# mom-ocean/MOM6

Measured on AMD Instinct MI355X. Metric: simulated-days/wall-sec, higher is better.
Workload: dtype f64

## Files before the change

mom6_amd/csrc/barotropic.hip:

```cpp
#include <algorithm>
#include <type_traits>
#include <vector>
#include <cmath>
#include "mom6x_dev.h"

void halo_wrap(mom6x_ctx *c, double *const *fields, const int *staggers, const int *nks, int n);

enum BTW {
  W_q = 0, W_DCor_u, W_DCor_v, W_gtot_E, W_gtot_W, W_gtot_N, W_gtot_S, W_eta, W_eta_PF,
  W_Cor_ref_u, W_Cor_ref_v, W_BT_force_u, W_BT_force_v, W_ubt, W_vbt, W_bt_rem_u, W_bt_rem_v,
  W_uhbt0, W_vhbt0, W_ubt_Cor, W_vbt_Cor, W_uhbt, W_vhbt, W_u_accel_bt, W_v_accel_bt,
  W_eta_src, W_e_anom, W_eta_sum, W_eta_wtd, W_ubt_wtd, W_vbt_wtd, W_eta_pred,
  W_uh0sum, W_vh0sum, W_ubt0, W_vbt0,
  W_f4u, W_f4u_2, W_f4u_3, W_f4u_4, W_f4v, W_f4v_2, W_f4v_3, W_f4v_4,
  W_BTCu,
  W_BTCv = W_BTCu + 10,
  W_BTtmp = W_BTCv + 10,
  W_uhn = W_BTtmp + 12,
  W_vhn,
  W_ubt2, W_vbt2, W_eta_pred2,
  W_COUNT
};

enum BTC { B_FA_EE = 0, B_FA_E0, B_FA_W0, B_FA_WW, B_uBT_WW, B_uBT_EE, B_crvW, B_crvE, B_uh_WW, B_uh_EE };
// ... 119 lines not shown
        if (e_k <= D_shallow) hat = h_harm;
        else {
          const double wt_arith = (e_k - D_shallow) / (h_arith + h_neglect);
          hat = wt_arith * h_arith + (1.0 - wt_arith) * h_harm;
        }
      }
      fr[c + k * slab] = hat;
      hattot = hattot + hat;
      e_below = e_k;
    }
    const double Ihattot = mC / (hattot + h_neglect);
    for (int k = 0; k < nz; k++) fr[c + k * slab] = fr[c + k * slab] * Ihattot;
  }
}

__global__ void k_bt_mass_source(Dm d, const double *__restrict__ G, const double *__restrict__ h,
                                 const double *__restrict__ eta, double *eta_cor, int set_cor, double Z_to_H) {
  const int i = blockIdx.x * blockDim.x + threadIdx.x, j = blockIdx.y * blockDim.y + threadIdx.y;
  if (i > d.ni - 1 || j > d.nj - 1) return;
  const size_t c = ix2(d, i, j);
  double eta_h = h[c] - gm(G, d, MOM6X_G_bathyT)[c] * Z_to_H;
  for (int k = 1; k < d.nk; k++) eta_h = eta_h + h[c + (size_t)k * d.slab];
  const double d_eta = eta_h - eta[c];
  eta_cor[c] = set_cor ? d_eta : (eta_cor[c] + d_eta);
}

__global__ void k_bt_mass_source_from(Dm d, const double *__restrict__ eta_h, const double *__restrict__ eta, double *eta_cor, int set_cor) {
  const int i = blockIdx.x * blockDim.x + threadIdx.x, j = blockIdx.y * blockDim.y + threadIdx.y;
  if (i > d.ni - 1 || j > d.nj - 1) return;
  const size_t c = ix2(d, i, j);
  const double d_eta = eta_h[c] - eta[c];
  eta_cor[c] = set_cor ? d_eta : (eta_cor[c] + d_eta);
}

__global__ void k_set_dtbt(Dm d, const double *__restrict__ G, const double *__restrict__ pbce,
                           const double *__restrict__ frhatu, const double *__restrict__ frhatv,
                           double gtot_est, double Z_to_H, double zadd, int add_max, double bebt, double cor_scale2,
                           double *Idt_max2_out, const double *__restrict__ eta) {
  const int i = blockIdx.x * blockDim.x + threadIdx.x, j = blockIdx.y * blockDim.y + threadIdx.y;
  if (i > d.ni - 1 || j > d.nj - 1) return;
  const int st = d.pitch;
  const size_t c = ix2(d, i, j), slab = (size_t)d.slab;
  const double *bathyT = gm(G, d, MOM6X_G_bathyT), *dy_Cu = gm(G, d, MOM6X_G_dy_Cu), *dx_Cv = gm(G, d, MOM6X_G_dx_Cv);
  const double *IdxCu = gm(G, d, MOM6X_G_IdxCu), *IdyCv = gm(G, d, MOM6X_G_IdyCv), *f2 = gm(G, d, MOM6X_G_Coriolis2Bu);
  double DatuE, DatuW, DatvN, DatvS;
  if (add_max) {
    DatuE = dy_Cu[c] * Z_to_H * dmax(dmax(bathyT[c + 1], bathyT[c]) + zadd, 0.0);
    DatuW = dy_Cu[c - 1] * Z_to_H * dmax(dmax(bathyT[c], bathyT[c - 1]) + zadd, 0.0);
    DatvN = dx_Cv[c] * Z_to_H * dmax(dmax(bathyT[c + st], bathyT[c]) + zadd, 0.0);
    DatvS = dx_Cv[c - st] * Z_to_H * dmax(dmax(bathyT[c], bathyT[c - st]) + zadd, 0.0);
  } else {
    auto Hc = [&](size_t x) { return eta ? (bathyT[x] * Z_to_H + eta[x]) : ((bathyT[x] + zadd) * Z_to_H); };
    const double H0 = Hc(c), HE = Hc(c + 1), HW = Hc(c - 1);
    const double HN = Hc(c + st), HS = Hc(c - st);
    DatuE = 0.0; if ((H0 > 0.0) && (HE > 0.0)) DatuE = dy_Cu[c] * (2.0 * H0 * HE) / (H0 + HE);
    DatuW = 0.0; if ((HW > 0.0) && (H0 > 0.0)) DatuW = dy_Cu[c - 1] * (2.0 * HW * H0) / (HW + H0);
    DatvN = 0.0; if ((H0 > 0.0) && (HN > 0.0)) DatvN = dx_Cv[c] * (2.0 * H0 * HN) / (H0 + HN);
    DatvS = 0.0; if ((HS > 0.0) && (H0 > 0.0)) DatvS = dx_Cv[c - st] * (2.0 * HS * H0) / (HS + H0);
  }
  double gE = gtot_est, gW = gtot_est, gN = gtot_est, gS = gtot_est;
  if (pbce) {
    gE = gW = gN = gS = 0.0;
    for (int k = 0; k < d.nk; k++) {
      const double pb = pbce[c + k * slab];
      gE = gE + pb * frhatu[c + k * slab];
      gW = gW + pb * frhatu[c - 1 + k * slab];
      gN = gN + pb * frhatv[c + k * slab];
      gS = gS + pb * frhatv[c - st + k * slab];
    }
  }
  Idt_max2_out[c] = 0.5 * (1.0 + 2.0 * bebt) * (gm(G, d, MOM6X_G_IareaT)[c] *
      (((gE * DatuE * IdxCu[c]) + (gW * DatuW * IdxCu[c - 1])) + ((gN * DatvN * IdyCv[c]) + (gS * DatvS * IdyCv[c - st]))) +
      ((f2[c] + f2[c - 1 - st]) + (f2[c - 1] + f2[c - st])) * cor_scale2);
}

struct ColArgs {
  const double *visc_rem, *frhat, *U_Cor, *pbce, *uh0, *u_uh0, *U_in, *bc_accel, *tau, *tau_bot, *IDat;
  const double *hf; double h_neglect;
  double *ubt_Cor, *gtot_m , *gtot_p , *uh0sum, *ubt0, *ubt, *BT_force, *bt_rem;
  double Instep, RZ_to_H, vel_underflow;
  int nstep, wt_uv_bug, visc_rem_u_uh0, strong_drag;
};

template <int DIR, bool HF>
__global__ void __launch_bounds__(256)
k_bt_col(Dm d, const double *__restrict__ G, ColArgs A) {
  const int i = I_BASE((DIR ? 0 : -1)) + blockIdx.x * blockDim.x + threadIdx.x;
  const int j = (DIR ? -1 : 0) + blockIdx.y * blockDim.y + threadIdx.y;
  if (i > d.ni - 1 || j > d.nj - 1) return;
  if (i < ((DIR ? 0 : -1))) return;
  const int st = DIR ? d.pitch : 1, nz = d.nk;
  const size_t c = ix2(d, i, j), slab = (size_t)d.slab;
  const double subroundoff = 1e-30;
  const double mC = gm(G, d, DIR ? MOM6X_G_mask2dCv : MOM6X_G_mask2dCu)[c];
  double Ihattot = 0.0;
  if (HF) {
    double hattot = 0.0;
    for (int k = 0; k < nz; k++) hattot = hattot + A.hf[c + (size_t)k * slab];
    Ihattot = mC / (hattot + A.h_neglect);
  }
#define FRH(k) (HF ? A.hf[c + (size_t)(k) * slab] * Ihattot : A.frhat[c + (size_t)(k) * slab])
  double Iwt_tot = 1.0;
  if (!A.wt_uv_bug) {
    double tot = 0.0;
    for (int k = 0; k < nz; k++) {
      double vr = dmin(A.visc_rem[c + k * slab], 1.);
      vr = dmax(vr, 1. - 0.5 * A.Instep / (vr + subroundoff));
      vr = dmax(vr, 0.);
      const double w = FRH(k) * vr;
      tot = (k == 0) ? w : (tot + w);
    }
    Iwt_tot = tot;
    if (fabs(tot) > 0.0) Iwt_tot = mC / tot;
  }
  double ubt_Cor = 0.0, gm_ = 0.0, gp_ = 0.0, uh0sum = 0.0, ubt0 = 0.0, ubt = 0.0, av_rem = 0.0;
  double BT_force = 0.0;
  if (mC > 0.0) {
    BT_force = A.tau[c] * A.RZ_to_H * A.IDat[c] * A.visc_rem[c];
    if (A.tau_bot) BT_force = BT_force - A.tau_bot[c] * A.RZ_to_H * A.IDat[c];
  }
  for (int k = 0; k < nz; k++) {
    const size_t f = c + k * slab;
    const double vrem = A.visc_rem[f], frh = FRH(k);
    double vr = dmin(vrem, 1.);
    vr = dmax(vr, 1. - 0.5 * A.Instep / (vr + subroundoff));
    vr = dmax(vr, 0.);
    double wt = frh * vr;
    if (!A.wt_uv_bug) wt = wt * Iwt_tot;
    ubt_Cor = ubt_Cor + wt * A.U_Cor[f];
    gm_ = gm_ + A.pbce[f] * wt;
    gp_ = gp_ + A.pbce[f + st] * wt;
    if (A.uh0) {
      uh0sum = uh0sum + A.uh0[f];
      ubt0 = ubt0 + (A.visc_rem_u_uh0 ? wt : frh) * A.u_uh0[f];
    }
    ubt = ubt + wt * A.U_in[f];
    BT_force = BT_force + wt * A.bc_accel[f];
    av_rem = av_rem + frh * vrem;
  }
#undef FRH
  A.ubt_Cor[c] = ubt_Cor;
  A.gtot_m[c] = gm_;
  A.gtot_p[c + st] = gp_;
  if (A.uh0) { A.uh0sum[c] = uh0sum; A.ubt0[c] = ubt0; }
  if (fabs(ubt) < A.vel_underflow) ubt = 0.0;
  A.ubt[c] = ubt;
  A.BT_force[c] = BT_force;
  double bt_rem;
  if (A.strong_drag) {
    bt_rem = mC * ((A.nstep * av_rem) / (1.0 + (A.nstep - 1) * av_rem));
  } else {
    bt_rem = 0.0;
    if (mC * av_rem > 0.0) bt_rem = mC * pow(av_rem, A.Instep);
  }
  A.bt_rem[c] = bt_rem;
}

__global__ void k_btcont_copy(Dm d, mom6x_BT_cont BT, double *tmp) {
  const int i = -1 + blockIdx.x * blockDim.x + threadIdx.x;
  const int j = -1 + blockIdx.y * blockDim.y + threadIdx.y;
  if (i > d.ni - 1 || j > d.nj - 1) return;
  const size_t c = ix2(d, i, j), slab = (size_t)d.slab;
  if (j >= 0) {
    tmp[0 * slab + c] = BT.uBT_EE[c]; tmp[1 * slab + c] = BT.uBT_WW[c]; tmp[2 * slab + c] = BT.FA_u_EE[c];
    tmp[3 * slab + c] = BT.FA_u_E0[c]; tmp[4 * slab + c] = BT.FA_u_W0[c]; tmp[5 * slab + c] = BT.FA_u_WW[c];
  }
  if (i >= 0) {
    tmp[6 * slab + c] = BT.vBT_NN[c]; tmp[7 * slab + c] = BT.vBT_SS[c]; tmp[8 * slab + c] = BT.FA_v_NN[c];
    tmp[9 * slab + c] = BT.FA_v_N0[c]; tmp[10 * slab + c] = BT.FA_v_S0[c]; tmp[11 * slab + c] = BT.FA_v_SS[c];
  }
}
__global__ void k_face_areas_as_fits(Dm d, const double *__restrict__ G, double Z_ref, double Z_to_H, double *tmp, const double *__restrict__ eta) {
  const int i = -2 + blockIdx.x * blockDim.x + threadIdx.x;
  const int j = -2 + blockIdx.y * blockDim.y + threadIdx.y;
  if (i > d.ni || j > d.nj) return;
  const int st = d.pitch;
  const size_t c = ix2(d, i, j), slab = (size_t)d.slab;
  const double *bathyT = gm(G, d, MOM6X_G_bathyT);
  const double H1 = eta ? (bathyT[c] * Z_to_H + eta[c]) : ((bathyT[c] + Z_ref) * Z_to_H);
  if (j >= -1) {
    const double H2 = eta ? (bathyT[c + 1] * Z_to_H + eta[c + 1]) : ((bathyT[c + 1] + Z_ref) * Z_to_H);
    double Dat = 0.0;
    if ((H1 > 0.0) && (H2 > 0.0)) Dat = gm(G, d, MOM6X_G_dy_Cu)[c] * (2.0 * H1 * H2) / (H1 + H2);
    tmp[0 * slab + c] = -1.0e100; tmp[1 * slab + c] = 1.0e100;
    tmp[2 * slab + c] = Dat; tmp[3 * slab + c] = Dat; tmp[4 * slab + c] = Dat; tmp[5 * slab + c] = Dat;
  }
  if (i >= -1) {
    const double H2 = eta ? (bathyT[c + st] * Z_to_H + eta[c + st]) : ((bathyT[c + st] + Z_ref) * Z_to_H);
    double Dat = 0.0;
    if ((H1 > 0.0) && (H2 > 0.0)) Dat = gm(G, d, MOM6X_G_dx_Cv)[c] * (2.0 * H1 * H2) / (H1 + H2);
    tmp[6 * slab + c] = -1.0e100; tmp[7 * slab + c] = 1.0e100;
    tmp[8 * slab + c] = Dat; tmp[9 * slab + c] = Dat; tmp[10 * slab + c] = Dat; tmp[11 * slab + c] = Dat;
  }
}
__global__ void k_face_areas_eta(Dm d, const double *__restrict__ G, double Z_to_H, const double *__restrict__ eta, double *Bu, double *Bv,
                                 int isv, int iev, int jsv, int jev) {
  const int i = isv - 2 + blockIdx.x * blockDim.x + threadIdx.x;
  const int j = jsv - 2 + blockIdx.y * blockDim.y + threadIdx.y;
  if (i > iev + 1 || j > jev + 1) return;
  const int st = d.pitch;
  const size_t c = ix2(d, i, j), slab = (size_t)d.slab;
  const double *bathyT = gm(G, d, MOM6X_G_bathyT);
  const double H1 = bathyT[c] * Z_to_H + eta[c];
  if (j >= jsv - 1) {
    const double H2 = bathyT[c + 1] * Z_to_H + eta[c + 1];
    double Dat = 0.0;
    if ((H1 > 0.0) && (H2 > 0.0)) Dat = gm(G, d, MOM6X_G_dy_Cu)[c] * (2.0 * H1 * H2) / (H1 + H2);
    Bu[B_FA_EE * slab + c] = Dat; Bu[B_FA_E0 * slab + c] = Dat; Bu[B_FA_W0 * slab + c] = Dat; Bu[B_FA_WW * slab + c] = Dat;
  }
  if (i >= isv - 1) {
    const double H2 = bathyT[c + st] * Z_to_H + eta[c + st];
    double Dat = 0.0;
    if ((H1 > 0.0) && (H2 > 0.0)) Dat = gm(G, d, MOM6X_G_dx_Cv)[c] * (2.0 * H1 * H2) / (H1 + H2);
    Bv[B_FA_EE * slab + c] = Dat; Bv[B_FA_E0 * slab + c] = Dat; Bv[B_FA_W0 * slab + c] = Dat; Bv[B_FA_WW * slab + c] = Dat;
  }
}
__global__ void k_btcl(Dm d, const double *__restrict__ tmp, double *Bu, double *Bv, int hs) {
  const int i = -hs - 1 + blockIdx.x * blockDim.x + threadIdx.x;
  const int j = -hs - 1 + blockIdx.y * blockDim.y + threadIdx.y;
  if (i > d.ni - 1 + hs || j > d.nj - 1 + hs) return;
  const size_t c = ix2(d, i, j), slab = (size_t)d.slab;
  const double C1_3 = 1.0 / 3.0;
  for (int dir = 0; dir < 2; dir++) {
    if (dir == 0 && j < -hs) continue;
    if (dir == 1 && i < -hs) continue;
    const double *t = tmp + (size_t)(dir * 6) * slab;
    double *B = dir ? Bv : Bu;
    const double FA_EE = t[2 * slab + c], FA_E0 = t[3 * slab + c], FA_W0 = t[4 * slab + c], FA_WW = t[5 * slab + c];
    const double uBT_EE = 1.0 * t[0 * slab + c], uBT_WW = 1.0 * t[1 * slab + c];
    B[B_FA_EE * slab + c] = FA_EE; B[B_FA_E0 * slab + c] = FA_E0; B[B_FA_W0 * slab + c] = FA_W0; B[B_FA_WW * slab + c] = FA_WW;
    B[B_uBT_EE * slab + c] = uBT_EE; B[B_uBT_WW * slab + c] = uBT_WW;
    B[B_uh_EE * slab + c] = uBT_EE * (C1_3 * (2.0 * FA_E0 + FA_EE));
    B[B_uh_WW * slab + c] = uBT_WW * (C1_3 * (2.0 * FA_W0 + FA_WW));
    double crvW = 0.0, crvE = 0.0;
    if (fabs(uBT_WW) > 0.0) crvW = (C1_3 * (FA_WW - FA_W0)) / (uBT_WW * uBT_WW);
    if (fabs(uBT_EE) > 0.0) crvE = (C1_3 * (FA_EE - FA_E0)) / (uBT_EE * uBT_EE);
    B[B_crvW * slab + c] = crvW; B[B_crvE * slab + c] = crvE;
  }
// ... 371 lines not shown
                               dtA * ((s_un[ty][tx - 1] - s_un[ty][tx]) + (s_vn[ty - 1][tx] - s_vn[ty][tx]));
      work[(size_t)P.e_out * slab + c] = eta_PF_BT;
      if (A.find_etaav && (fabs(A.wt_accel2_next) > 0.0) && i >= 0 && i <= d.ni - 1 && j >= 0 && j <= d.nj - 1)
        work[W_eta_sum * slab + c] = work[W_eta_sum * slab + c] + A.wt_accel2_next * eta_PF_BT;
    }
    if (i >= 0 && i < d.ni && j >= 0 && j < d.nj) {
      const double bT = gm(G, d, MOM6X_G_bathyT)[c];
      if ((e < -Z_to_H * bT) && (gm(G, d, MOM6X_G_mask2dT)[c] > 0.0)) {
        atomicAdd(&warn[0], 1ULL);
        if (atomicCAS(&warn[1], 0ULL, 1ULL) == 0ULL) { warn_info[0] = e; warn_info[1] = -bT; warn_info[2] = (double)i; warn_info[3] = (double)j; }
      }
    }
  }
}

__global__ void k_bt_clip(Dm d, const double *__restrict__ G, double *work, double dt, double CFL_trunc,
                          int isv, int iev, int jsv, int jev) {
  const int i = isv - 1 + blockIdx.x * blockDim.x + threadIdx.x;
  const int j = jsv - 1 + blockIdx.y * blockDim.y + threadIdx.y;
  if (i > iev || j > jev) return;
  const int st = d.pitch;
  const size_t c = ix2(d, i, j), slab = (size_t)d.slab;
  const double *IareaT = gm(G, d, MOM6X_G_IareaT), *areaT = gm(G, d, MOM6X_G_areaT);
  if (j >= jsv) {
    const double dy = gm(G, d, MOM6X_G_dy_Cu)[c];
    double u = work[W_ubt * slab + c];
    if ((u * (dt * dy)) * IareaT[c + 1] < -CFL_trunc) u = (-0.95 * CFL_trunc) * (areaT[c + 1] / (dt * dy));
    else if ((u * (dt * dy)) * IareaT[c] > CFL_trunc) u = (0.95 * CFL_trunc) * (areaT[c] / (dt * dy));
    work[W_ubt * slab + c] = u;
  }
  if (i >= isv) {
    const double dx = gm(G, d, MOM6X_G_dx_Cv)[c];
    double v = work[W_vbt * slab + c];
    if ((v * (dt * dx)) * IareaT[c + st] < -CFL_trunc) v = (-0.9 * CFL_trunc) * (areaT[c + st] / (dt * dx));
    else if ((v * (dt * dx)) * IareaT[c] > CFL_trunc) v = (0.9 * CFL_trunc) * (areaT[c] / (dt * dx));
    work[W_vbt * slab + c] = v;
  }
}

__global__ void k_bt_post(Dm d, double *work, const double *__restrict__ eta_in, double *eta_out, double *etaav,
                          double dgeo_de, double I_sum_wt_accel, double I_sum_wt_eta) {
  const int i = blockIdx.x * blockDim.x + threadIdx.x, j = blockIdx.y * blockDim.y + threadIdx.y;
  if (i > d.ni - 1 || j > d.nj - 1) return;
  const size_t c = ix2(d, i, j), slab = (size_t)d.slab;
  if (etaav) etaav[c] = work[W_eta_sum * slab + c] * I_sum_wt_accel;
  work[W_e_anom * slab + c] = dgeo_de * (0.5 * (work[W_eta * slab + c] + eta_in[c]) - work[W_eta_PF * slab + c]);
  eta_out[c] = work[W_eta_wtd * slab + c] * I_sum_wt_eta;
}

__global__ void __launch_bounds__(256)
k_layer_accel(Dm d, const double *__restrict__ G, const double *__restrict__ work, const double *__restrict__ pbce,
              double *__restrict__ accel_layer_u, double *__restrict__ accel_layer_v, double accel_underflow) {
  const int i = I_BASE(-1) + blockIdx.x * blockDim.x + threadIdx.x;
  const int j = -1 + blockIdx.y * blockDim.y + threadIdx.y;
  if (i > d.ni - 1 || j > d.nj - 1) return;
  if (i < (-1)) return;
  const int st = d.pitch;
  const size_t c = ix2(d, i, j), slab = (size_t)d.slab;
  const int k0 = blockIdx.z * KCHUNK, k1 = min(k0 + KCHUNK, d.nk);
  const double *e_anom = work + W_e_anom * slab;
  const double ea = e_anom[c], ea_E = e_anom[c + 1], ea_N = e_anom[c + st];
  const double g_E = work[W_gtot_E * slab + c], g_W = work[W_gtot_W * slab + c + 1];
  const double g_N = work[W_gtot_N * slab + c], g_S = work[W_gtot_S * slab + c + st];
  const double ua = work[W_u_accel_bt * slab + c], va = work[W_v_accel_bt * slab + c];
  const double IdxCu = gm(G, d, MOM6X_G_IdxCu)[c], IdyCv = gm(G, d, MOM6X_G_IdyCv)[c];
  for (int k = k0; k < k1; k++) {
    const size_t c3 = c + (size_t)k * slab;
    const double pb = pbce[c3];
    if (j >= 0) {
      double a = (ua - (((pbce[c3 + 1] - g_W) * ea_E) - ((pb - g_E) * ea)) * IdxCu);
      if (fabs(a) < accel_underflow) a = 0.0;
      accel_layer_u[c3] = a;
    }
    if (i >= 0) {
      double a = (va - (((pbce[c3 + st] - g_S) * ea_N) - ((pb - g_N) * ea)) * IdyCv);
      if (fabs(a) < accel_underflow) a = 0.0;
      accel_layer_v[c3] = a;
    }
  }
}

}

void bt_defer_layer_accel(mom6x_ctx *c, bool on) { if (c->bts) c->bts->la_defer = on; }

void bt_defer_btcalc(mom6x_ctx *c, bool on) {
  static const bool eager = [] { const char *e = getenv("MOM6X_BTCALC"); return e && !strcmp(e, "eager"); }();
  if (c->bts) c->bts->fr_defer = on && !eager;
}
static void btcalc_from_faces(mom6x_ctx *c, const double *h_u, const double *h_v) {
  const Dm d = c->d;
  const dim3 b = blk2();
  if (d.nk <= COLS_NK_BOUND) {
#define BTC(NKT) do {                                                                                                                   \
    KLAUNCH(c, "k_btcalc<0>", (k_btcalc_cols<0, NKT>), grid3(nxa(d.ni + 1, -1), d.nj, 1, b), b, d, c->G, h_u, c->bts->frhatu, c->GV.H_subroundoff); \
    KLAUNCH(c, "k_btcalc<1>", (k_btcalc_cols<1, NKT>), grid3(d.ni, d.nj + 1, 1, b), b, d, c->G, h_v, c->bts->frhatv, c->GV.H_subroundoff); } while (0)
    COLS_NK_DISPATCH(d.nk, BTC);
#undef BTC
    return;
  }
  KLAUNCH(c, "k_btcalc<0>", k_btcalc<0>, grid3(nxa(d.ni + 1, -1), d.nj, 1, b), b, d, c->G, (const double *)nullptr, h_u, c->bts->frhatu,
          c->GV.H_subroundoff, c->GV.Z_to_H, 0);
  KLAUNCH(c, "k_btcalc<1>", k_btcalc<1>, grid3(d.ni, d.nj + 1, 1, b), b, d, c->G, (const double *)nullptr, h_v, c->bts->frhatv,
          c->GV.H_subroundoff, c->GV.Z_to_H, 0);
}
int bt_frhat_materialize(mom6x_ctx *c) {
  BTState *s = c->bts;
  if (!s || !s->fr_pending) return MOM6X_OK;
  HIPCHK(hipSetDevice(c->device));
  btcalc_from_faces(c, s->fr_hu, s->fr_hv);
  s->fr_pending = false;
  HIPCHK(hipGetLastError());
  return MOM6X_OK;
}

bool bt_layer_accel_src(mom6x_ctx *c, LayerAccelSrc *u, LayerAccelSrc *v) {
  BTState *s = c->bts;
  if (!s || !s->la_pending) return false;
  const size_t slab = (size_t)c->d.slab;
  const double *w = s->work;
  u->pbce = v->pbce = s->la_pbce; u->e_anom = v->e_anom = w + W_e_anom * slab;
  u->g_own = w + W_gtot_E * slab; u->g_nbr = w + W_gtot_W * slab; u->a2d = w + W_u_accel_bt * slab;
  v->g_own = w + W_gtot_N * slab; v->g_nbr = w + W_gtot_S * slab; v->a2d = w + W_v_accel_bt * slab;
  u->underflow = v->underflow = s->la_underflow;
  return true;
}

int bt_layer_accel_materialize(mom6x_ctx *c, double *accel_layer_u, double *accel_layer_v) {
  BTState *s = c->bts;
  REQUIRE(s && s->la_pending, MOM6X_EINVAL, "btstep_layer_accel: the deferred layer accelerations of the step's last btstep are gone "
          "(another btstep has run since)");
  HIPCHK(hipSetDevice(c->device));
  const Dm d = c->d;
  const dim3 b = blk2();
  KLAUNCH(c, "k_layer_accel", k_layer_accel, grid3(nxa(d.ni + 1, -1), d.nj + 1, nchunks(d.nk), b), b, d, c->G, (const double *)s->work,
          s->la_pbce, accel_layer_u, accel_layer_v, s->la_underflow);
  s->la_pending = false;
  HIPCHK(hipGetLastError());
  return MOM6X_OK;
}

void bt_state_free(mom6x_ctx *c) {
  if (!c->bts) return;
  BTState *s = c->bts;
  double *ptrs[] = { s->frhatu, s->frhatv, s->IDatu, s->IDatv, s->ubtav, s->vbtav, s->eta_cor, s->q_D, s->D_u_Cor,
                     s->D_v_Cor, s->work, s->warn_info };
  for (double *p : ptrs) (void)hipFree(p);
  (void)hipFree(s->warn);
  delete s;
  c->bts = nullptr;
}

extern "C" int mom6x_btstep_warnings(mom6x_ctx *c, int reset, long long *count, double *info) {
  REQUIRE(c && c->bts && count, MOM6X_EINVAL, "mom6x_btstep_warnings: barotropic_init has not been called");
  HIPCHK(hipSetDevice(c->device));
  HIPCHK(hipStreamSynchronize(c->stream));
  unsigned long long w[2];
  HIPCHK(hipMemcpy(w, c->bts->warn, sizeof(w), hipMemcpyDeviceToHost));
  *count = (long long)w[0];
  if (info) HIPCHK(hipMemcpy(info, c->bts->warn_info, 4 * sizeof(double), hipMemcpyDeviceToHost));
  if (reset) HIPCHK(hipMemset(c->bts->warn, 0, sizeof(w)));
  return MOM6X_OK;
}

extern "C" int mom6x_barotropic_init(mom6x_ctx *c, const mom6x_barotropic_params *p) {
  REQUIRE(c && p, MOM6X_EINVAL, "mom6x_barotropic_init: null argument");
// ... 119 lines not shown
  const Dm d = c->d;
  const dim3 b = blk2();
  BTState *s = c->bts;
  { const int rcm = bt_frhat_materialize(c); if (rcm) return rcm; }
  double *tmp = s->work + (size_t)W_eta_pred * d.slab;
  HIPCHK(hipMemsetAsync(tmp, 0, sizeof(double) * d.slab, c->stream));
  KLAUNCH(c, "k_set_dtbt", k_set_dtbt, grid3(d.ni, d.nj, 1, b), b, d, c->G, pbce, s->frhatu, s->frhatv, gtot_est,
                     c->GV.Z_to_H, c->bt.Z_ref + SSH_add, add_max, c->bt.bebt, c->bt.BT_Coriolis_scale * c->bt.BT_Coriolis_scale, tmp, eta);
  HIPCHK(hipGetLastError());
  std::vector<double> host((size_t)d.slab);
  HIPCHK(hipMemcpyAsync(host.data(), tmp, sizeof(double) * d.slab, hipMemcpyDeviceToHost, c->stream));
  HIPCHK(hipStreamSynchronize(c->stream));
  double min_max_dt2 = 1.0e38;
  for (int j = 0; j < d.nj; j++) for (int i = 0; i < d.ni; i++) {
    const double I2 = host[(size_t)(i + d.ioff) + (size_t)(j + d.joff) * d.pitch];
    if (I2 * min_max_dt2 > 1.0) min_max_dt2 = 1.0 / I2;
  }
  const double dgeo_de = 1.0 + fmax(0.0, c->bt.G_extra);
  double dtbt_max = sqrt(min_max_dt2 / dgeo_de);
  { int rc_ = comm_allreduce_scalar(c, &dtbt_max, 0); if (rc_) return rc_; }
  c->bt.dtbt = c->bt.dtbt_fraction * dtbt_max;
  if (dtbt_out) *dtbt_out = c->bt.dtbt;
  return MOM6X_OK;
}

extern "C" int mom6x_btstep(mom6x_ctx *c, const double *U_in, const double *V_in, const double *eta_in, double dt,
                            const double *bc_accel_u, const double *bc_accel_v, const double *taux, const double *tauy,
                            const double *pbce, const double *eta_PF_in, const double *U_Cor, const double *V_Cor,
                            double *accel_layer_u, double *accel_layer_v, double *eta_out, double *uhbtav,
                            double *vhbtav, const double *visc_rem_u, const double *visc_rem_v,
                            const mom6x_BT_cont *BT_cont, const double *taux_bot, const double *tauy_bot,
                            const double *uh0, const double *vh0, const double *u_uh0, const double *v_vh0,
                            double *etaav) {
  REQUIRE(c && c->bt_init, MOM6X_EINVAL, "btstep: Module MOM_barotropic must be initialized before it is used.");
  REQUIRE(U_in && V_in && eta_in && bc_accel_u && bc_accel_v && taux && tauy && pbce && eta_PF_in && U_Cor && V_Cor &&
          accel_layer_u && accel_layer_v && eta_out && uhbtav && vhbtav && visc_rem_u && visc_rem_v,
          MOM6X_EINVAL, "btstep: null mandatory array");
  const bool add_uh0 = (uh0 != nullptr);
  REQUIRE(!add_uh0 || (vh0 && u_uh0 && v_vh0), MOM6X_EINVAL,
          "btstep: vh0, u_uh0, and v_vh0 must be associated if uh0 is used.");
  REQUIRE((taux_bot != nullptr) == (tauy_bot != nullptr), MOM6X_EINVAL, "btstep: taux_bot and tauy_bot come together");
  HIPCHK(hipSetDevice(c->device));
  const Dm d = c->d;
  const mom6x_barotropic_params &P = c->bt;
  BTState *s = c->bts;
  double *work = s->work;
  const size_t slab = (size_t)d.slab;
  const dim3 b = blk2();
  hipStream_t st = c->stream;
  const int is = 0, ie = d.ni - 1, js = 0, je = d.nj - 1;

  const double Idt = 1.0 / dt;
  const bool evolving_face_areas = !BT_cont && P.nonlinear_continuity && P.nonlin_cont_update_period > 0;
  const int stencil = evolving_face_areas ? std::max(2, P.min_stencil) : ((P.min_stencil > 1) ? P.min_stencil : 1);
  const int num_cycles = (P.use_wide_halos && d.halo / stencil >= 1) ? d.halo / stencil : 1;
  const int isvf = is - (num_cycles - 1) * stencil, ievf = ie + (num_cycles - 1) * stencil;
  const int jsvf = js - (num_cycles - 1) * stencil, jevf = je + (num_cycles - 1) * stencil;
  REQUIRE(P.dtbt > 0.0, MOM6X_EINVAL, "btstep: dtbt must be positive (call set_dtbt or set params.dtbt)");
  const int nstep = (int)ceil(dt / P.dtbt - 0.0001);
  s->nstep_last = nstep;
  const double Instep = 1.0 / (double)nstep;
  const double dtbt = dt * Instep;
  const double dgeo_de = 1.0 + P.G_extra;

  HIPCHK(hipMemsetAsync(work, 0, (size_t)W_COUNT * slab * sizeof(double), st));
  KLAUNCH(c, "k_bt_copy_in", k_bt_copy_in, grid3(d.ni + 2 * d.halo + 1, d.nj + 2 * d.halo + 1, 1, b), b, d, work, eta_in,
                     eta_PF_in, s->q_D, s->D_u_Cor, s->D_v_Cor);

  ColArgs Au;
  memset(&Au, 0, sizeof(Au));
  Au.visc_rem = visc_rem_u; Au.frhat = s->frhatu; Au.U_Cor = U_Cor; Au.pbce = pbce; Au.uh0 = uh0; Au.u_uh0 = u_uh0;
  Au.U_in = U_in; Au.bc_accel = bc_accel_u; Au.tau = taux; Au.tau_bot = taux_bot; Au.IDat = s->IDatu;
  Au.ubt_Cor = work + W_ubt_Cor * slab; Au.gtot_m = work + W_gtot_E * slab; Au.gtot_p = work + W_gtot_W * slab;
  Au.uh0sum = work + W_uh0sum * slab; Au.ubt0 = work + W_ubt0 * slab; Au.ubt = work + W_ubt * slab;
  Au.BT_force = work + W_BT_force_u * slab; Au.bt_rem = work + W_bt_rem_u * slab;
  Au.Instep = Instep; Au.RZ_to_H = c->GV.RZ_to_H; Au.vel_underflow = P.vel_underflow; Au.nstep = nstep;
  Au.wt_uv_bug = P.wt_uv_bug; Au.visc_rem_u_uh0 = P.visc_rem_u_uh0; Au.strong_drag = P.strong_drag;
  ColArgs Av = Au;
  Av.visc_rem = visc_rem_v; Av.frhat = s->frhatv; Av.U_Cor = V_Cor; Av.uh0 = vh0; Av.u_uh0 = v_vh0; Av.U_in = V_in;
  Av.bc_accel = bc_accel_v; Av.tau = tauy; Av.tau_bot = tauy_bot; Av.IDat = s->IDatv;
  Av.ubt_Cor = work + W_vbt_Cor * slab; Av.gtot_m = work + W_gtot_N * slab; Av.gtot_p = work + W_gtot_S * slab;
  Av.uh0sum = work + W_vh0sum * slab; Av.ubt0 = work + W_vbt0 * slab; Av.ubt = work + W_vbt * slab;
  Av.BT_force = work + W_BT_force_v * slab; Av.bt_rem = work + W_bt_rem_v * slab;
  if (s->fr_pending) {
    Au.hf = s->fr_hu; Av.hf = s->fr_hv; Au.h_neglect = Av.h_neglect = c->GV.H_subroundoff;
    KLAUNCH(c, "k_bt_col<0>", (k_bt_col<0, true>), grid3(nxa(d.ni + 1, -1), d.nj, 1, b), b, d, c->G, Au);
    KLAUNCH(c, "k_bt_col<1>", (k_bt_col<1, true>), grid3(d.ni, d.nj + 1, 1, b), b, d, c->G, Av);
  } else {
    { const int rcm = bt_frhat_materialize(c); if (rcm) return rcm; }
    KLAUNCH(c, "k_bt_col<0>", (k_bt_col<0, false>), grid3(nxa(d.ni + 1, -1), d.nj, 1, b), b, d, c->G, Au);
    KLAUNCH(c, "k_bt_col<1>", (k_bt_col<1, false>), grid3(d.ni, d.nj + 1, 1, b), b, d, c->G, Av);
  }

  double *tmp = work + W_BTtmp * slab;
  if (BT_cont) KLAUNCH(c, "k_btcont_copy", k_btcont_copy, grid3(d.ni + 1, d.nj + 1, 1, b), b, d, *BT_cont, tmp);
  else KLAUNCH(c, "k_face_areas_as_fits", k_face_areas_as_fits, grid3(d.ni + 3, d.nj + 3, 1, b), b, d, c->G, P.Z_ref, c->GV.Z_to_H, tmp,
               P.nonlinear_continuity ? (const double *)(work + W_eta * slab) : (const double *)nullptr);
  {
    double *f[18]; int stg[18], nks[18];
    for (int m = 0; m < 12; m++) { f[m] = tmp + (size_t)m * slab; stg[m] = (m < 6) ? 1 : 2; nks[m] = 1; }
    double *g[] = { work + W_gtot_E * slab, work + W_gtot_N * slab, work + W_gtot_W * slab, work + W_gtot_S * slab,
                    work + W_ubt_Cor * slab, work + W_vbt_Cor * slab };
    const int gs[] = { 0, 0, 0, 0, 1, 2 };
    for (int m = 0; m < 6; m++) { f[12 + m] = g[m]; stg[12 + m] = gs[m]; nks[12 + m] = 1; }
    halo_wrap(c, f, stg, nks, 18);
  }
  const int hs = 1 + ievf - ie;
  KLAUNCH(c, "k_btcl", k_btcl, grid3(d.ni + 2 * hs + 1, d.nj + 2 * hs + 1, 1, b), b, d, tmp, work + W_BTCu * slab,
                     work + W_BTCv * slab, hs);
  if (add_uh0) KLAUNCH(c, "k_uhbt0", k_uhbt0, grid3(d.ni + 1, d.nj + 1, 1, b), b, d, work, work);

  KLAUNCH(c, "k_find_Cor", k_find_Cor, grid3(ievf - isvf + 3, jevf - jsvf + 3, 1, b), b, d, work, P.Sadourny, isvf, ievf, jsvf, jevf);
  KLAUNCH(c, "k_cor_ref_eta_src", k_cor_ref_eta_src, grid3(d.ni + 1, d.nj + 1, 1, b), b, d, c->G, work, s->eta_cor, Instep,
                     P.bound_BT_corr ? ((BT_cont && P.BT_cont_bounds) ? 1 : 2) : 0, P.maxCFL_BT_cont * Idt, dt, c->GV.Z_to_H, P.Z_ref, P.maxvel);
  {
    std::vector<double *> f = { work + W_eta_PF * slab, work + W_eta_src * slab, work + W_bt_rem_u * slab, work + W_bt_rem_v * slab,
                                work + W_BT_force_u * slab, work + W_BT_force_v * slab };
    std::vector<int> stg = { 0, 0, 1, 2, 1, 2 };
    if (add_uh0) { f.push_back(work + W_uhbt0 * slab); stg.push_back(1); f.push_back(work + W_vhbt0 * slab); stg.push_back(2); }
    f.push_back(work + W_Cor_ref_u * slab); stg.push_back(1); f.push_back(work + W_Cor_ref_v * slab); stg.push_back(2);
    std::vector<int> nks(f.size(), 1);
    halo_wrap(c, f.data(), stg.data(), nks.data(), (int)f.size());
  }

  double dt_filt;
  if (P.dt_bt_filter >= 0.0) dt_filt = 0.5 * fmax(0.0, fmin(P.dt_bt_filter, 2.0 * dt));
  else dt_filt = 0.5 * fmax(0.0, dt * fmin(-P.dt_bt_filter, 2.0));
  const int nfilter = (int)ceil(dt_filt / dtbt);
  const int nt = nstep + nfilter;
  REQUIRE(nt > 0, MOM6X_EINVAL, "btstep: number of barotropic step (nstep+nfilter) is 0");
  std::vector<double> wt_vel(nt + 2, 0.0), wt_eta(nt + 2, 0.0), wt_trans(nt + 2, 0.0), wt_accel(nt + 2, 0.0), wt_accel2(nt + 2, 0.0);
  double sum_wt_vel = 0.0, sum_wt_eta = 0.0, sum_wt_accel = 0.0, sum_wt_trans = 0.0;
  for (int n = 1; n <= nt; n++) {
    if ((n == nstep) || (dt_filt - abs(n - nstep) * dtbt >= 0.0)) { wt_vel[n] = 1.0; wt_eta[n] = 1.0; }
    else if (dtbt + dt_filt - abs(n - nstep) * dtbt > 0.0) { wt_vel[n] = 1.0 + (dt_filt / dtbt) - abs(n - nstep); wt_eta[n] = wt_vel[n]; }
    else { wt_vel[n] = 0.0; wt_eta[n] = 0.0; }
    sum_wt_vel = sum_wt_vel + wt_vel[n]; sum_wt_eta = sum_wt_eta + wt_eta[n];
  }
  for (int n = nt; n >= 1; n--) {
    wt_trans[n] = wt_trans[n + 1] + wt_eta[n];
    wt_accel[n] = wt_accel[n + 1] + wt_vel[n];
    sum_wt_accel = sum_wt_accel + wt_accel[n]; sum_wt_trans = sum_wt_trans + wt_trans[n];
  }
  const double I_sum_wt_vel = 1.0 / sum_wt_vel, I_sum_wt_accel = 1.0 / sum_wt_accel;
  const double I_sum_wt_eta = 1.0 / sum_wt_eta, I_sum_wt_trans = 1.0 / sum_wt_trans;
  for (int n = 1; n <= nt; n++) {
    wt_vel[n] = wt_vel[n] * I_sum_wt_vel;
    wt_accel2[n] = wt_accel[n] * I_sum_wt_accel;
    wt_trans[n] = wt_trans[n] * I_sum_wt_trans;
    wt_accel[n] = wt_accel[n] * I_sum_wt_accel;
    wt_eta[n] = wt_eta[n] * I_sum_wt_eta;
  }

  HIPCHK(hipMemsetAsync(s->ubtav, 0, slab * sizeof(double), st));
  HIPCHK(hipMemsetAsync(s->vbtav, 0, slab * sizeof(double), st));
  HIPCHK(hipMemsetAsync(uhbtav, 0, slab * sizeof(double), st));
  HIPCHK(hipMemsetAsync(vhbtav, 0, slab * sizeof(double), st));
  LoopArgs L;
  memset(&L, 0, sizeof(L));
  L.dtbt = dtbt; L.dgeo_de = dgeo_de; L.vel_underflow = P.vel_underflow;
  if (P.BT_project_velocity) { L.trans_wt1 = (1.0 + P.bebt); L.trans_wt2 = -P.bebt; }
  else { L.trans_wt1 = P.bebt; L.trans_wt2 = (1.0 - P.bebt); }
  L.project = P.BT_project_velocity; L.find_etaav = (etaav != nullptr);
  L.f4_on_the_fly = 1; L.Sadourny = P.Sadourny;
  int isv = is, iev = ie, jsv = js, jev = je;
  const bool pass_uhn = !P.clip_velocity && !P.BT_project_velocity && !evolving_face_areas;
  L.store_uhn = pass_uhn ? 1 : 0;
  static const int substep_env = [] { const char *e = getenv("MOM6X_BT_SUBSTEP"); return !e ? 0 : (!strcmp(e, "kernels") ? 1 : (!strcmp(e, "fused") ? 2 : 0)); }();
  const bool small_tile = ((long)d.ni * d.nj <= 512L * 1024L);
  const bool fused = pass_uhn && (substep_env == 2 || (substep_env == 0 && small_tile));
  const bool overlap_loop = fused && c->bt_overlap && halo_can_overlap(c) && d.ni >= 96 && d.nj >= 32;
  SubPlanes SP = { W_ubt, fused ? W_ubt2 : W_ubt, W_vbt, fused ? W_vbt2 : W_vbt, W_eta_pred, fused ? W_eta_pred2 : W_eta_pred };
  const int loop_stg[] = { 0, 1, 2, 1, 2 }, loop_nk[] = { 1, 1, 1, 1, 1 };
  bool pred_done = false;
  for (int n = 1; n <= nt; n++) {
// ... 85 lines not shown
```

Before: 0.1928.

## Add register-cached, software-pipelined column kernel for barotropic layer sums

Adds a k_bt_col_cols kernel, templated on a compile-time layer bound, that keeps frhat/hf and visc_rem columns in registers instead of re-reading them in each of the two vertical passes. The remaining per-layer inputs are prefetched in double-buffered groups of four, with sched barriers so loads overlap the accumulation. It also skips the separate u_uh0 load when that pointer aliases U_in or U_Cor. It runs by default when nk is within the column bound, with 64-thread blocks. The cost is higher register pressure and more template instantiations, and an env var keeps the old walking kernel available.

Result: no change. 0.1942 (median of 6 runs) (+0.7%).

```diff
diff --git a/mom6_amd/csrc/barotropic.hip b/mom6_amd/csrc/barotropic.hip
--- a/mom6_amd/csrc/barotropic.hip
+++ b/mom6_amd/csrc/barotropic.hip
@@ -225,6 +225,66 @@
   int nstep, wt_uv_bug, visc_rem_u_uh0, strong_drag;
 };
 
+struct BtColSums {
+  double ubt_Cor, gm_, gp_, uh0sum, ubt0, ubt, BT_force, av_rem;
+  __device__ __forceinline__ static double vr_of(double vrem, double Instep) {
+    const double subroundoff = 1e-30;
+    double vr = dmin(vrem, 1.);
+    vr = dmax(vr, 1. - 0.5 * Instep / (vr + subroundoff));
+    vr = dmax(vr, 0.);
+    return vr;
+  }
+  __device__ __forceinline__ static double wt_tot_next(double tot, int k, double frh, double vrem, double Instep) {
+    const double w = frh * vr_of(vrem, Instep);
+    return (k == 0) ? w : (tot + w);
+  }
+  __device__ __forceinline__ static double Iwt_tot_of(double tot, double mC) {
+    double Iwt_tot = tot;
+    if (fabs(tot) > 0.0) Iwt_tot = mC / tot;
+    return Iwt_tot;
+  }
+  __device__ __forceinline__ void start(const ColArgs &A, size_t c, double mC, double vrem0) {
+    ubt_Cor = 0.0; gm_ = 0.0; gp_ = 0.0; uh0sum = 0.0; ubt0 = 0.0; ubt = 0.0; av_rem = 0.0;
+    BT_force = 0.0;
+    if (mC > 0.0) {
+      BT_force = A.tau[c] * A.RZ_to_H * A.IDat[c] * vrem0;
+      if (A.tau_bot) BT_force = BT_force - A.tau_bot[c] * A.RZ_to_H * A.IDat[c];
+    }
+  }
+  __device__ __forceinline__ void layer(const ColArgs &A, double Iwt_tot, double frh, double vrem, double U_Cor, double pb_m, double pb_p,
+                                        double uh0, double u_uh0, double U_in, double bc_accel) {
+    double wt = frh * vr_of(vrem, A.Instep);
+    if (!A.wt_uv_bug) wt = wt * Iwt_tot;
+    ubt_Cor = ubt_Cor + wt * U_Cor;
+    gm_ = gm_ + pb_m * wt;
+    gp_ = gp_ + pb_p * wt;
+    if (A.uh0) {
+      uh0sum = uh0sum + uh0;
+      ubt0 = ubt0 + (A.visc_rem_u_uh0 ? wt : frh) * u_uh0;
+    }
+    ubt = ubt + wt * U_in;
+    BT_force = BT_force + wt * bc_accel;
+    av_rem = av_rem + frh * vrem;
+  }
+  __device__ __forceinline__ void store(const ColArgs &A, size_t c, int st, double mC) {
+    A.ubt_Cor[c] = ubt_Cor;
+    A.gtot_m[c] = gm_;
+    A.gtot_p[c + st] = gp_;
+    if (A.uh0) { A.uh0sum[c] = uh0sum; A.ubt0[c] = ubt0; }
+    if (fabs(ubt) < A.vel_underflow) ubt = 0.0;
+    A.ubt[c] = ubt;
+    A.BT_force[c] = BT_force;
+    double bt_rem;
+    if (A.strong_drag) {
+      bt_rem = mC * ((A.nstep * av_rem) / (1.0 + (A.nstep - 1) * av_rem));
+    } else {
+      bt_rem = 0.0;
+      if (mC * av_rem > 0.0) bt_rem = mC * pow(av_rem, A.Instep);
+    }
+    A.bt_rem[c] = bt_rem;
+  }
+};
+
 template <int DIR, bool HF>
 __global__ void __launch_bounds__(256)
 k_bt_col(Dm d, const double *__restrict__ G, ColArgs A) {
@@ -234,7 +294,6 @@
   if (i < ((DIR ? 0 : -1))) return;
   const int st = DIR ? d.pitch : 1, nz = d.nk;
   const size_t c = ix2(d, i, j), slab = (size_t)d.slab;
-  const double subroundoff = 1e-30;
   const double mC = gm(G, d, DIR ? MOM6X_G_mask2dCv : MOM6X_G_mask2dCu)[c];
   double Ihattot = 0.0;
   if (HF) {
@@ -246,57 +305,97 @@
   double Iwt_tot = 1.0;
   if (!A.wt_uv_bug) {
     double tot = 0.0;
-    for (int k = 0; k < nz; k++) {
-      double vr = dmin(A.visc_rem[c + k * slab], 1.);
-      vr = dmax(vr, 1. - 0.5 * A.Instep / (vr + subroundoff));
-      vr = dmax(vr, 0.);
-      const double w = FRH(k) * vr;
-      tot = (k == 0) ? w : (tot + w);
-    }
-    Iwt_tot = tot;
-    if (fabs(tot) > 0.0) Iwt_tot = mC / tot;
-  }
-  double ubt_Cor = 0.0, gm_ = 0.0, gp_ = 0.0, uh0sum = 0.0, ubt0 = 0.0, ubt = 0.0, av_rem = 0.0;
-  double BT_force = 0.0;
-  if (mC > 0.0) {
-    BT_force = A.tau[c] * A.RZ_to_H * A.IDat[c] * A.visc_rem[c];
-    if (A.tau_bot) BT_force = BT_force - A.tau_bot[c] * A.RZ_to_H * A.IDat[c];
-  }
+    for (int k = 0; k < nz; k++) tot = BtColSums::wt_tot_next(tot, k, FRH(k), A.visc_rem[c + k * slab], A.Instep);
+    Iwt_tot = BtColSums::Iwt_tot_of(tot, mC);
+  }
+  BtColSums S;
+  S.start(A, c, mC, A.visc_rem[c]);
   for (int k = 0; k < nz; k++) {
     const size_t f = c + k * slab;
-    const double vrem = A.visc_rem[f], frh = FRH(k);
-    double vr = dmin(vrem, 1.);
-    vr = dmax(vr, 1. - 0.5 * A.Instep / (vr + subroundoff));
-    vr = dmax(vr, 0.);
-    double wt = frh * vr;
-    if (!A.wt_uv_bug) wt = wt * Iwt_tot;
-    ubt_Cor = ubt_Cor + wt * A.U_Cor[f];
-    gm_ = gm_ + A.pbce[f] * wt;
-    gp_ = gp_ + A.pbce[f + st] * wt;
-    if (A.uh0) {
-      uh0sum = uh0sum + A.uh0[f];
-      ubt0 = ubt0 + (A.visc_rem_u_uh0 ? wt : frh) * A.u_uh0[f];
-    }
-    ubt = ubt + wt * A.U_in[f];
-    BT_force = BT_force + wt * A.bc_accel[f];
-    av_rem = av_rem + frh * vrem;
+    S.layer(A, Iwt_tot, FRH(k), A.visc_rem[f], A.U_Cor[f], A.pbce[f], A.pbce[f + st], A.uh0 ? A.uh0[f] : 0.0, A.uh0 ? A.u_uh0[f] : 0.0,
+            A.U_in[f], A.bc_accel[f]);
   }
 #undef FRH
-  A.ubt_Cor[c] = ubt_Cor;
-  A.gtot_m[c] = gm_;
-  A.gtot_p[c + st] = gp_;
-  if (A.uh0) { A.uh0sum[c] = uh0sum; A.ubt0[c] = ubt0; }
-  if (fabs(ubt) < A.vel_underflow) ubt = 0.0;
-  A.ubt[c] = ubt;
-  A.BT_force[c] = BT_force;
-  double bt_rem;
-  if (A.strong_drag) {
-    bt_rem = mC * ((A.nstep * av_rem) / (1.0 + (A.nstep - 1) * av_rem));
-  } else {
-    bt_rem = 0.0;
-    if (mC * av_rem > 0.0) bt_rem = mC * pow(av_rem, A.Instep);
-  }
-  A.bt_rem[c] = bt_rem;
+  S.store(A, c, st, mC);
+}
+
+template <int DIR, bool HF, int NKT>
+__global__ void __launch_bounds__(64)
+k_bt_col_cols(Dm d, const double *__restrict__ G, ColArgs A, int st) {
+  constexpr int NK = NK_OF(NKT);
+  const int nk = d.nk;
+  const int i = I_BASE((DIR ? 0 : -1)) + blockIdx.x * 64 + threadIdx.x;
+  const int j = (DIR ? -1 : 0) + blockIdx.y;
+  if (i > d.ni - 1 || j > d.nj - 1) return;
+  if (i < ((DIR ? 0 : -1))) return;
+  const size_t c = ix2(d, i, j), slab = (size_t)d.slab;
+  const double mC = gm(G, d, DIR ? MOM6X_G_mask2dCv : MOM6X_G_mask2dCu)[c];
+  const double *__restrict__ fsrc = HF ? A.hf : A.frhat;
+  double fh[NK], vm[NK];
+#pragma unroll
+  for (int k = 0; k < NK; k++) if (k < nk) fh[k] = fsrc[c + (size_t)k * slab];
+#pragma unroll
+  for (int k = 0; k < NK; k++) if (k < nk) vm[k] = A.visc_rem[c + (size_t)k * slab];
+  const bool has_uh0 = A.uh0 != nullptr;
+  const bool uu_is_in = A.u_uh0 == A.U_in, uu_is_cor = A.u_uh0 == A.U_Cor;
+  const bool uu_own = has_uh0 && !uu_is_in && !uu_is_cor;
+  constexpr int BC_G = 4;
+  constexpr int NG = (NK + BC_G - 1) / BC_G;
+  double q_c[2][BC_G], q_m[2][BC_G], q_p[2][BC_G], q_h[2][BC_G], q_w[2][BC_G], q_i[2][BC_G], q_b[2][BC_G];
+  auto fetch = [&](int g, int b) {
+#pragma unroll
+    for (int m = 0; m < BC_G; m++) {
+      const int k = g * BC_G + m;
+      if (k < NK && k < nk) {
+        const size_t f = c + (size_t)k * slab;
+        q_c[b][m] = A.U_Cor[f];
+        q_m[b][m] = A.pbce[f];
+        q_p[b][m] = A.pbce[f + st];
+        if (has_uh0) q_h[b][m] = A.uh0[f];
+        if (uu_own) q_w[b][m] = A.u_uh0[f];
+        q_i[b][m] = A.U_in[f];
+        q_b[b][m] = A.bc_accel[f];
+      }
+    }
+  };
+  fetch(0, 0);
+  __builtin_amdgcn_sched_barrier(0);
+  double Ihattot = 0.0;
+  if (HF) {
+    double hattot = 0.0;
+#pragma unroll
+    for (int k = 0; k < NK; k++) if (k < nk) hattot = hattot + fh[k];
+    Ihattot = mC / (hattot + A.h_neglect);
+  }
+#define FRH(k) (HF ? fh[k] * Ihattot : fh[k])
+  double Iwt_tot = 1.0;
+  if (!A.wt_uv_bug) {
+    double tot = 0.0;
+#pragma unroll
+    for (int k = 0; k < NK; k++) if (k < nk) tot = BtColSums::wt_tot_next(tot, k, FRH(k), vm[k], A.Instep);
+    Iwt_tot = BtColSums::Iwt_tot_of(tot, mC);
+  }
+  BtColSums S;
+  S.start(A, c, mC, vm[0]);
+  __builtin_amdgcn_sched_barrier(0);
+#pragma unroll
+  for (int g = 0; g < NG; g++) {
+    if (g + 1 < NG) fetch(g + 1, (g + 1) & 1);
+    __builtin_amdgcn_sched_barrier(0);
+#pragma unroll
+    for (int m = 0; m < BC_G; m++) {
+      const int k = g * BC_G + m;
+      if (k < NK && k < nk) {
+        const double U_Cor = q_c[g & 1][m], U_in = q_i[g & 1][m];
+        const double uh0 = has_uh0 ? q_h[g & 1][m] : 0.0;
+        const double u_uh0 = uu_is_in ? U_in : (uu_is_cor ? U_Cor : (has_uh0 ? q_w[g & 1][m] : 0.0));
+        S.layer(A, Iwt_tot, FRH(k), vm[k], U_Cor, q_m[g & 1][m], q_p[g & 1][m], uh0, u_uh0, U_in, q_b[g & 1][m]);
+      }
+    }
+    __builtin_amdgcn_sched_barrier(0);
+  }
+#undef FRH
+  S.store(A, c, st, mC);
 }
 
 __global__ void k_btcont_copy(Dm d, mom6x_BT_cont BT, double *tmp) {
@@ -834,6 +933,11 @@
 
 }
 
+static bool bt_col_walk() {
+  static const bool walk = [] { const char *e = getenv("MOM6X_BT_COL"); return e && !strcmp(e, "walk"); }();
+  return walk;
+}
+
 void bt_defer_layer_accel(mom6x_ctx *c, bool on) { if (c->bts) c->bts->la_defer = on; }
 
 void bt_defer_btcalc(mom6x_ctx *c, bool on) {
@@ -1119,15 +1223,32 @@
   Av.ubt_Cor = work + W_vbt_Cor * slab; Av.gtot_m = work + W_gtot_N * slab; Av.gtot_p = work + W_gtot_S * slab;
   Av.uh0sum = work + W_vh0sum * slab; Av.ubt0 = work + W_vbt0 * slab; Av.ubt = work + W_vbt * slab;
   Av.BT_force = work + W_BT_force_v * slab; Av.bt_rem = work + W_bt_rem_v * slab;
+  const bool col_cols = d.nk <= COLS_NK_BOUND && !bt_col_walk();
+  const dim3 bcc(64, 1, 1);
+  const dim3 gu = grid3(nxa(d.ni + 1, -1), d.nj, 1, col_cols ? bcc : b), gv = grid3(d.ni, d.nj + 1, 1, col_cols ? bcc : b);
+#define BCC_T(NKT) do { KLAUNCH(c, "k_bt_col_cols<0>", (k_bt_col_cols<0, true, NKT>), gu, bcc, d, c->G, Au, 1);                                   \
+                        KLAUNCH(c, "k_bt_col_cols<1>", (k_bt_col_cols<1, true, NKT>), gv, bcc, d, c->G, Av, d.pitch); } while (0)
+#define BCC_F(NKT) do { KLAUNCH(c, "k_bt_col_cols<0>", (k_bt_col_cols<0, false, NKT>), gu, bcc, d, c->G, Au, 1);                                  \
+                        KLAUNCH(c, "k_bt_col_cols<1>", (k_bt_col_cols<1, false, NKT>), gv, bcc, d, c->G, Av, d.pitch); } while (0)
   if (s->fr_pending) {
     Au.hf = s->fr_hu; Av.hf = s->fr_hv; Au.h_neglect = Av.h_neglect = c->GV.H_subroundoff;
-    KLAUNCH(c, "k_bt_col<0>", (k_bt_col<0, true>), grid3(nxa(d.ni + 1, -1), d.nj, 1, b), b, d, c->G, Au);
-    KLAUNCH(c, "k_bt_col<1>", (k_bt_col<1, true>), grid3(d.ni, d.nj + 1, 1, b), b, d, c->G, Av);
+    if (col_cols) {
+      COLS_NK_DISPATCH(d.nk, BCC_T);
+    } else {
+      KLAUNCH(c, "k_bt_col<0>", (k_bt_col<0, true>), gu, b, d, c->G, Au);
+      KLAUNCH(c, "k_bt_col<1>", (k_bt_col<1, true>), gv, b, d, c->G, Av);
+    }
   } else {
     { const int rcm = bt_frhat_materialize(c); if (rcm) return rcm; }
-    KLAUNCH(c, "k_bt_col<0>", (k_bt_col<0, false>), grid3(nxa(d.ni + 1, -1), d.nj, 1, b), b, d, c->G, Au);
-    KLAUNCH(c, "k_bt_col<1>", (k_bt_col<1, false>), grid3(d.ni, d.nj + 1, 1, b), b, d, c->G, Av);
-  }
+    if (col_cols) {
+      COLS_NK_DISPATCH(d.nk, BCC_F);
+    } else {
+      KLAUNCH(c, "k_bt_col<0>", (k_bt_col<0, false>), gu, b, d, c->G, Au);
+      KLAUNCH(c, "k_bt_col<1>", (k_bt_col<1, false>), gv, b, d, c->G, Av);
+    }
+  }
+#undef BCC_T
+#undef BCC_F
 
   double *tmp = work + W_BTtmp * slab;
   if (BT_cont) KLAUNCH(c, "k_btcont_copy", k_btcont_copy, grid3(d.ni + 1, d.nj + 1, 1, b), b, d, *BT_cont, tmp);
```
